# zarr-developers/zarr-python

Measured on AMD Instinct MI355X. Metric: decoded GiB/s (device-resident), sharded 256^3 f32 64^3 chunks, 1/2/4/8 GPU, higher is better.
Workload: dtype u8

## Files before the change

include/zarrhip.h:

```cpp
#ifndef ZARRHIP_H
#define ZARRHIP_H

#include <stdint.h>

#ifdef __cplusplus
extern "C" {
#endif

#define ZHIP_ABI_VERSION 1
#define ZHIP_MAX_DIMS 8

#define ZHIP_OK 0
#define ZHIP_E_INVALID -1
#define ZHIP_E_HIP -2
#define ZHIP_E_UNSUPPORTED -3
#define ZHIP_E_IO -4
#define ZHIP_E_BOUNDS -5

#define ZHIP_ST_OK 0u
#define ZHIP_ST_MISSING 1u
#define ZHIP_ST_CRC_MISMATCH 2u
#define ZHIP_ST_INDEX_OOB 3u
#define ZHIP_ST_LENGTH_MISMATCH 4u

// ... 377 lines not shown
typedef struct zhip_value_op {
    uint32_t encode;
    uint32_t array_dt;
    uint32_t stored_dt;
    uint32_t stages;
    uint64_t offset, scale;
    uint32_t rounding;
    uint32_t out_of_range;
    uint32_t n_map;
    uint32_t fill_nan;
    uint64_t map_key[ZHIP_VALUE_MAX_MAP];
    uint64_t map_val[ZHIP_VALUE_MAX_MAP];
    uint64_t fill;
} zhip_value_op;

#define ZHIP_VI_MISSING 1u
#define ZHIP_VI_STATUS 2u

typedef struct zhip_value_dim {
    int64_t sa, sb;
    uint32_t count;
    uint32_t _pad;
    zhip_fdiv div;
} zhip_value_dim;

typedef struct zhip_value_item {
    int64_t a_base, b_base;
    uint32_t ndim;
    uint32_t total;
    uint32_t flags;
    uint32_t status;
    zhip_value_dim dims[ZHIP_MAX_DIMS];
} zhip_value_item;

int zhip_value_map(const zhip_value_op *op, const zhip_value_item *d_items, uint32_t n_items,
                   const uint32_t *d_tile_prefix, uint32_t n_tiles, const zhip_status *d_status,
                   const void *a, uint64_t a_size, void *b, uint64_t b_size, uint32_t *d_err,
                   uint32_t *d_nonempty, void *stream);
int zhip_emulate_value_map(const zhip_value_op *op, const zhip_value_item *items, uint32_t n_items,
                           const uint32_t *tile_prefix, uint32_t n_tiles, const zhip_status *status,
                           uint32_t n_status, const void *a, uint64_t a_size, void *b, uint64_t b_size,
                           uint32_t *err, uint32_t *nonempty);

int zhip_emulate_fill_eq(uint32_t itemsize, uint32_t lflags, const void *fill, const void *items,
                         uint64_t n_items, uint8_t *eq, uint32_t *fill_nan);

uint32_t zhip_crc32c_host(const void *data, uint64_t nbytes);

int zhip_selftest(void);
uint32_t zhip_emulate_chunk_crc(const zhip_plan *plan, const uint8_t *data);
uint32_t zhip_emulate_chunk_crc_pair(const zhip_plan *plan, const uint8_t *data);
uint32_t zhip_emulate_chunk_crc_il(const zhip_plan *plan, const uint8_t *data);
uint32_t zhip_emulate_chunk_crc_xw(const zhip_plan *plan, const uint8_t *data);
uint64_t zhip_plan_table_image(const zhip_plan *plan, int which, uint32_t *out, uint64_t cap);
uint32_t zhip_plan_table_offsets(const zhip_plan *plan, uint64_t *out, uint32_t cap);
uint32_t zhip_fdiv_eval(uint32_t n, uint32_t d);

#ifdef __cplusplus
}
#endif

#endif
```

zarr-python_amd/csrc/capi.cpp:

```cpp
#include <hip/hip_runtime.h>

#include <algorithm>
#include <climits>
#include <cstdio>
#include <cstdlib>
#include <cstring>
#include <new>
#include <string>
#include <vector>

#include "../../include/zarrhip.h"
#include "zhip_gf2.h"
#include "zhip_internal.h"
#include "zhip_axis.h"
#include "zhip_fill_eq.h"
#include "zhip_points.h"
#include "zhip_select.h"
#include "zhip_values.h"

using namespace zhip;

namespace {

thread_local std::string g_err;
// ... 1228 lines not shown
                acc = ap(0, acc ^ w[0]) ^ ap(1, w[1]) ^ ap(2, w[2]) ^ ap(3, w[3]);
            }
            unit ^= gf_mul(acc, h[T.kthread.off + t]);
        }
        V ^= gf_mul(unit, h[T.kunit.off + s]);
    }
    return ~(gf_mul(V, plan->c_inv) ^ plan->c3);
}

uint32_t zhip_emulate_chunk_crc_pair(const zhip_plan* plan, const uint8_t* data) {
    auto mulx = [](uint32_t b) { return (b >> 1) ^ (kPoly & (0u - (b & 1u))); };
    auto lanemul3 = [&](uint32_t a, uint32_t k) {
        uint32_t m3[8], m2[4];
        const uint32_t k1 = mulx(k), k2 = mulx(k1);
        for (uint32_t v = 0; v < 8; ++v) m3[v] = ((v & 4u) ? k : 0u) ^ ((v & 2u) ? k1 : 0u) ^ ((v & 1u) ? k2 : 0u);
        for (uint32_t v = 0; v < 4; ++v) m2[v] = ((v & 2u) ? k : 0u) ^ ((v & 1u) ? k1 : 0u);
        uint32_t p = m3[a & 7u];
        for (int j = 1; j < 10; ++j) p = mulx(mulx(mulx(p))) ^ m3[(a >> (3 * j)) & 7u];
        return mulx(mulx(p)) ^ m2[a >> 30];
    };
    const std::vector<uint32_t> h = build_row_tables(*plan);
    const TabSet& S = plan->tl.pair;
    return emulate_lanes(plan, data, &h[S.tab.off], &h[S.klane.off], S.klane.n, plan->kblocks,
                         [&](int64_t i, int64_t k) {
                             return (int64_t)plan->E - (i / kThreads + 1) * plan->seg + kWgStride * k + 16 * (i % kThreads);
                         },
                         lanemul3);
}

uint32_t zhip_emulate_chunk_crc_il(const zhip_plan* plan, const uint8_t* data) {
    if (!plan || !plan->il_S) return 0xFFFFFFFFu;
    const IlChoice c = il_choose(*plan, 0);
    const int64_t S = c.S, K = kDefaultBlocks;
    const int64_t lo_frame = (int64_t)plan->E - (int64_t)plan->nseg * K * kWgStride;
    const std::vector<uint32_t> h = build_row_tables(*plan);
    return emulate_lanes(plan, data, &h[c.set->tab.off], &h[c.set->klane.off], c.set->klane.n, (uint32_t)K,
                         [&](int64_t i, int64_t k) {
                             const int64_t r = i / kThreads, st0 = (r / S) * S * K + r % S;
                             return lo_frame + kWgStride * (st0 + S * k) + 16 * (i % kThreads);
                         },
                         [](uint32_t a, uint32_t k) { return gf_mul(a, k); });
}

uint32_t zhip_emulate_chunk_crc_xw(const zhip_plan* plan, const uint8_t* data) {
    if (!plan || !plan->xw_P) return 0xFFFFFFFFu;
    const int64_t lo_frame = (int64_t)plan->E - (int64_t)plan->nseg * kDefaultBlocks * kWgStride;
    const std::vector<uint32_t> h = build_row_tables(*plan);
    const TabSet& S = plan->tl.xw;
    return emulate_lanes(plan, data, &h[S.tab.off], &h[S.klane.off], S.klane.n, kDefaultBlocks,
                         [&](int64_t i, int64_t k) { return lo_frame + 8192 * (i / 64) + 1024 * k + 16 * (i % 64); },
                         [](uint32_t a, uint32_t k) { return gf_mul(a, k); });
}

int zhip_selftest(void) {
    const uint32_t* g_T = byte_tables().T;
    bool seen[256] = {false};
    for (int i = 0; i < 256; ++i) seen[g_T[i] >> 24] = true;
    for (int i = 0; i < 256; ++i)
        if (!seen[i]) return set_err(1, "T top-byte map is not a bijection");
    uint32_t v = 0x12345678u;
    for (int it = 0; it < 1000; ++it) {
        v = v * 1664525u + 1013904223u;
        const uint32_t a = (v >> 8) ^ g_T[v & 255u];
        if (a != gf_mul(v, xpow8(1))) return set_err(2, "A_1 != multiply by x^8");
        if (gf_mul(gf_mul(v, xpow8(777)), xpow8_inv(777)) != v) return set_err(3, "x^-8n inverse wrong");
    }
    if (crc_bytewise((const uint8_t*)"123456789", 9) != 0xE3069283u) return set_err(4, "check value");
    const uint32_t ds[] = {1, 2, 3, 5, 7, 10, 15, 60, 64, 100, 255, 256, 1000, 4096, 65537, 1000003u};
    for (uint32_t d : ds) {
        const zhip_fdiv f = make_fdiv(d);
        uint32_t x = 1;
        for (int it = 0; it < 20000; ++it) {
            x = x * 1103515245u + 12345u;
            const uint32_t n = (it < 1000) ? (uint32_t)it : (x & 0x7FFFFFFFu);
            if (fdiv_apply(n, f.m, f.s) != n / d) return set_err(5, "fdiv wrong");
        }
        const uint32_t nmax = 0x7FFFFFFFu;
        if (fdiv_apply(nmax, f.m, f.s) != nmax / d) return set_err(5, "fdiv wrong at 2^31-1");
    }
    const uint64_t sizes[] = {0, 1, 3, 4, 15, 16, 17, 100, 4095, 4096, 4097, 32768, 32769, 100000, 262148};
    std::vector<uint8_t> buf(262148);
    uint32_t r = 7;
    for (auto& b : buf) {
        r = r * 1664525u + 1013904223u;
        b = (uint8_t)(r >> 24);
    }
    for (uint64_t n : sizes) {
        zhip_layout L{};
        L.ndim = 1;
        L.itemsize = 1;
        L.shape[0] = (int32_t)n;
        L.nbytes = n;
        zhip_plan* p = nullptr;
        if (zhip_plan_create(&L, &p) != ZHIP_OK) return 6;
        const uint32_t got = zhip_emulate_chunk_crc(p, buf.data());
        const uint32_t got_pair = zhip_emulate_chunk_crc_pair(p, buf.data());
        zhip_plan_destroy(p);
        if (got != crc_bytewise(buf.data(), n)) return set_err(7, "emulated kernel CRC wrong at n=" + std::to_string(n));
        if (got_pair != crc_bytewise(buf.data(), n))
            return set_err(8, "emulated pair-kernel CRC wrong at n=" + std::to_string(n));
    }
    return 0;
}

}
```

zarr-python_amd/csrc/decode.hip:

```cpp
#include <hip/hip_runtime.h>

#include "../../include/zarrhip.h"
#include "zhip_gf2.h"
#include "zhip_internal.h"
#include "zhip_dispatch.h"
#include "zhip_device.h"
#include "zhip_decode_common.h"
#include "zhip_arrival.h"

namespace zhip {

#if ZHIP_TUNING
int g_tune_max_grid = 0;
#endif

template <bool CRC, bool WRITE, bool FAST, int ITEM, int SWAP, int K = 8>
__global__ __launch_bounds__(kThreads) void k_decode(const DecodeParams p) {
    __shared__ uint32_t s_tab[CRC ? 16 * 256 : 1];
    __shared__ uint32_t s_red[2][kThreads / 64];
    const int t = threadIdx.x;
    uint32_t kth = 0;
    const bool crc_on = CRC && !(p.tune & kTuneSkipCrc);
    if constexpr (CRC) {
        const uint4* g = reinterpret_cast<const uint4*>(p.horner);
// ... 546 lines not shown
        return select_il_kernel_arm(L.crc, L.item, L.swap, g_tune_arm);
    if (tune & kTuneCfLookup) return select_il_kernel_cf(L.crc, L.item, L.swap);
    if (tune & kTuneIlLean) return select_il_kernel_lean(L.crc, L.item, L.swap);
    if (tune & (kTuneIlRegMul | kTuneIlOcc6))
        return select_il_kernel_regmul(L.crc, L.item, L.swap, (tune & kTuneIlOcc6) != 0);
    if (tune & (kTuneNoTables | kTuneNoRunEnd | kTuneNoPub | kTuneStamp))
        return select_il_kernel_tuned(L.crc, L.item, L.swap);
#endif
    return select_il_kernel(L.crc, L.item, L.swap, L.p.aff_ok != 0);
}

static KernelFn pick_pair_kernel(const Launch& L, int nu) {
#if ZHIP_TUNING
    const uint32_t tune = L.tune;
    if (nu == 2 && !(tune & (kTuneTrailingCrc | kTuneSplitChain))) {
        KernelFn fn = (tune & kTuneSkipCrc) ? select_pair_kernel(L.crc, L.item, L.swap, kPairNoLookups)
                      : (tune & (kTunePrio | kTuneDeferB))
                          ? select_pair_kernel(L.crc, L.item, L.swap,
                                               (tune & kTunePrio) && (tune & kTuneDeferB) ? kPairPrioDeferB
                                               : (tune & kTunePrio) ? kPairPrio : kPairDeferB)
                          : nullptr;
        if (fn) return fn;
    }
#endif
    return select_pair_kernel(L.crc, L.item, L.swap, nu == 2 ? kPairTwo : kPairSingle);
}

static bool takes_lead4(const Launch& L) {
    return L.p.nseg == 1u && L.p.E <= 4u * kWgStride && g_tune_arm != kArmNoLead4;
}

static bool takes_lead(const Launch& L) { return !L.crc && L.p.n_idx; }

static bool takes_interleaved(const Launch& L) {
    const DecodeParams& p = L.p;
    return p.il_S != 0 && L.crc && !(L.tune & (kTuneNoIl | kTuneSkipCrc | kTuneSingle | kTuneDuo)) &&
           ((L.tune & kTuneIl) || p.il_S >= 8u);
}

static bool takes_ilh(const Launch& L, bool il) {
    const DecodeParams& p = L.p;
    return il && p.ilh_klane && p.n_units <= kIlwMaxUnits && L.lb_ok && p.nseg <= 32u &&
           (g_tune_arm == kArmProduction || g_tune_arm == kArmIlhProduction) && (L.tune & ~kTuneStamp) == 0;
}

static bool takes_ilw512(const Launch& L, bool il) {
    const DecodeParams& p = L.p;
    return il && p.ilw_nt == 512u && p.n_units <= kIlwMaxUnits &&
           (g_tune_arm == kArmProduction || g_tune_arm == kArmRowMap || g_tune_arm == kArmIlw512Small ||
            ((g_tune_arm == kArmSplitPub || g_tune_arm == kArmLookBack) && p.aff_ok)) &&
           (L.tune & ~kTuneStamp) == 0;
}

static int launch_row_units(const Launch& L) {
    const DecodeParams& p = L.p;
    const uint32_t tune = L.tune;
    const bool crc = L.crc;
    if (takes_lead4(L)) return launch_lead4(L);
    if (takes_lead(L)) return launch_lead(L);
    const bool il = takes_interleaved(L);
#if ZHIP_TUNING
    int rc;
    if (launch_row_arm(L, il, rc)) return rc;
#endif
    if (takes_ilh(L, il))
        return fire(select_ilh_kernel(L.item, L.swap, true, p.aff_ok != 0), "k_decode_ilh",
                    unit_grid(p, 2u * p.n_units), kThreads, p, L.stream);
    if (takes_ilw512(L, il)) {
        const IlwForm form = g_tune_arm == kArmSplitPub ? kIlw512Split
                             : (g_tune_arm == kArmLookBack && L.lb_ok && p.nseg <= 64u) ? kIlw512LookBack : kIlw512;
        return fire(select_ilw_kernel(L.item, L.swap, form, false, p.aff_ok != 0), "k_decode_ilw512",
                    unit_grid(p, p.n_units), 512, p, L.stream);
    }
    if (il) return fire(pick_il_kernel(L), "k_decode_il", unit_grid(p, p.n_units), kThreads, p, L.stream);
    const int nu = (tune & kTuneSingle) ? 1 : 2;
    KernelFn fn = pick_pair_kernel(L, nu);
    if (!fn) return ZHIP_E_UNSUPPORTED;
    if ((tune & kTuneDuo) || (p.nseg > 32 && !(tune & (kTuneSingle | kTuneSkipCrc))))
        return fire(select_duo_kernel(crc, L.item, L.swap), "k_decode_duo",
                    unit_grid(p, (uint32_t)(((uint64_t)p.n_units + 1u) / 2u)), 2 * kThreads, p, L.stream);
    const uint32_t grid = unit_grid(p, (uint32_t)(((uint64_t)p.n_units + nu - 1u) / nu));
    return fire(fn, "k_decode_pair", grid, kThreads, with_xcd_runs(L, grid, nu == 2), L.stream);
}

static int launch_persistent(const Launch& L, KernelFn fn, const char* name) {
    uint32_t grid = L.p.n_units;
    if (fn && grid) {
        const uint32_t resident = (uint32_t)resident_grid(fn, L.max_grid);
        if (grid > resident) grid = resident;
    }
    return fire(fn, name, grid, kThreads, L.p, L.stream);
}

static int launch_tile4(const Launch& L) {
    const DecodeParams& p = L.p;
    const bool f4 = ZHIP_TUNING && p.t4f_tab != nullptr && L.crc;
    const bool w4 = !f4 && p.t4w_tab != nullptr && L.crc;
    if (w4 && ((p.t2w_kq && g_tune_arm != kArmTileFour && g_tune_arm != kArmTile1w) ||
               (g_tune_arm == kArmTile1w && p.t1w_kq))) {
        const bool one = g_tune_arm == kArmTile1w;
        const Tile2wForm form = one ? kT2wOne : g_tune_arm == kArmSplitPub ? kT2wSplit
                                : (g_tune_arm == kArmTile2wByteTab && p.tbt_tab) ? kT2wByteTab : kT2wTwo;
        DecodeParams q = p;
        q.t4w_kq = one ? p.t1w_kq : p.t2w_kq;
        return fire(select_tile2w_kernel(L.item, L.swap, form),
                    one ? "k_decode_tile1w" : form == kT2wSplit ? "k_decode_tile2ws"
// ... 18 lines not shown
    const bool gw = p.t4w_tab != nullptr && L.crc;
    const bool defer = p.defer != 0 && g_tune_arm != kArmDeferred;
    TilegwForm form = (gw && p.t2w_kq && g_tune_arm != kArmTileFour && g_tune_arm != kArmDeferred &&
                       g_tune_arm != kArmTilegLanes) ? kTgwTwo : kTgwFour;
    const bool two = form == kTgwTwo;
#if ZHIP_TUNING
    if (gw && g_tune_arm == kArmTilegLanes && p.tglt_kq) form = kTgwLanes;
    if (two && g_tune_arm == kArmTilegPacked) form = kTgwPacked;
    if (two && g_tune_arm == kArmTilegLookBack && L.lb_ok && p.n_groups <= 128u) form = kTgwLookBack;
    if (two && g_tune_arm == kArmTilegByteTab && p.tbt_tab) form = kTgwByteTab;
#endif
    KernelFn fn = gw ? select_tilegw_kernel(L.item, L.swap, defer, form)
                     : select_tileg_kernel(L.crc, L.item, L.swap, defer);
    const uint64_t grid = (uint64_t)p.n_chunks * p.n_groups * (two ? 2u : 1u);
    if (grid >= (1ull << 31)) return ZHIP_E_UNSUPPORTED;
    DecodeParams q = p;
    if (two) q.t4w_kq = p.t2w_kq;
    if (form == kTgwLanes) q.t4w_kq = p.tglt_kq;
    return fire(fn, !gw ? "k_decode_tileg" : form == kTgwPacked ? "k_decode_tileg2wp"
                    : form == kTgwLookBack ? "k_decode_tileg2w_lb" : form == kTgwByteTab ? "k_decode_tileg2w_bt"
                    : two ? "k_decode_tileg2w" : form == kTgwLanes ? "k_decode_tileglt" : "k_decode_tilegw",
                (uint32_t)grid, kThreads, q, L.stream);
}

static Launch make_launch(const DecodeParams& p, hipStream_t stream, int max_grid) {
    const bool crc = (p.lflags & ZHIP_LF_CRC) != 0;
    const bool lb_ok = p.n_chunks < (uint32_t)(max_grid / 8);
    if (g_tune_max_grid > 0) max_grid = g_tune_max_grid;
    return {p, stream, max_grid, ZHIP_TUNING ? p.tune : 0u, lb_ok, crc, item_mode(p.lflags, (int)p.g.itemsize),
            p.g.itemsize};
}

static bool takes_row_units(const Launch& L) {
    const DecodeParams& p = L.p;
    const bool lead_launch = !L.crc && p.n_idx != 0;
    return p.rows && p.rowmap && p.seg == (uint32_t)kWgStride * kDefaultBlocks &&
           (!(L.tune & kTunePersist) || lead_launch);
}

static bool takes_plain_il(const Launch& L) {
    if (!takes_row_units(L) || takes_lead4(L) || takes_lead(L)) return false;
    const bool il = takes_interleaved(L);
    if (!il || takes_ilh(L, il) || takes_ilw512(L, il)) return false;
    return g_tune_arm == kArmProduction && L.tune == 0u;
}

uint64_t g_launch_count = 0;

int launch_decode_multi(const DecodeParams* ps, const int* max_grid, uint32_t n, hipStream_t stream, bool dry) {
    if (n < 2u || n > (uint32_t)ZHIP_MULTI_MAX) return ZHIP_E_UNSUPPORTED;
    MultiParams m{};
    MultiFn fn = nullptr;
    uint64_t total = 0;
    for (uint32_t i = 0; i < n; ++i) {
        const Launch L = make_launch(ps[i], stream, max_grid[i]);
        if (!takes_plain_il(L)) return ZHIP_E_UNSUPPORTED;
        MultiFn f = select_il_multi_kernel(L.crc, L.item, L.swap, ps[i].aff_ok != 0);
        if (!f || (i && f != fn)) return ZHIP_E_UNSUPPORTED;
        fn = f;
        const uint32_t grid = unit_grid(ps[i], ps[i].n_units);
        if (grid == 0) return ZHIP_E_UNSUPPORTED;
        m.q[i] = ps[i];
        m.g0[i] = (uint32_t)total;
        total += grid;
        if (total > 0x7FFFFFFFull) return ZHIP_E_UNSUPPORTED;
    }
    for (uint32_t i = n; i <= (uint32_t)ZHIP_MULTI_MAX; ++i) m.g0[i] = (uint32_t)total;
    m.n = n;
    if (dry) return ZHIP_OK;
    return fire(fn, "k_decode_il", (uint32_t)total, kThreads, m, stream);
}

int launch_decode(const DecodeParams& p, hipStream_t stream, int max_grid) {
    const Launch L = make_launch(p, stream, max_grid);
    const bool crc = L.crc;
    if (takes_row_units(L)) return launch_row_units(L);
    if (p.rows)
        return launch_persistent(L, select_rows_kernel(crc, L.item, L.swap, (int)(p.seg / kWgStride)), "k_decode_rows");
    if (p.tq >= 0 && p.tile4) return launch_tile4(L);
    if (p.tq >= 0 && p.tile2) return launch_tile_pairs(L);
    if (p.tq >= 0 && p.tileg) return launch_tile_groups(L);
    if (p.tq >= 0) return launch_persistent(L, select_tile_kernel(crc, L.item, L.swap), "k_decode_tile");
    return launch_persistent(L, select_decode_kernel(crc, (p.lflags & ZHIP_LF_NO_WRITE) == 0, p.fast != 0, L.item,
                                                     L.swap, (int)(p.seg / kWgStride)), "k_decode");
}

}

extern "C" const char* zhip_last_kernel(void) { return zhip::g_last_kernel; }
extern "C" uint32_t zhip_last_grid(void) { return zhip::g_last_grid; }
extern "C" uint64_t zhip_launch_count(void) { return zhip::g_launch_count; }
```

zarr-python_amd/csrc/decode_rows.hip:

```cpp
#include <hip/hip_runtime.h>

#include "../../include/zarrhip.h"
#include "zhip_gf2.h"
#include "zhip_internal.h"
#include "zhip_dispatch.h"
#include "zhip_device.h"
#include "zhip_decode_common.h"
#include "zhip_arrival.h"

namespace zhip {

namespace {

typedef unsigned int zhip_v4u_a1 __attribute__((ext_vector_type(4), aligned(1)));
typedef __attribute__((address_space(1))) const zhip_v4u_a1 zhip_gv4u_a1;

typedef __attribute__((address_space(1))) const uint32_t zhip_gu32_a1 __attribute__((aligned(1)));

__device__ __forceinline__ uint32_t load_u32_any(const uint8_t* a) {
    return *(zhip_gu32_a1*)(reinterpret_cast<uintptr_t>(a));
}

__device__ __forceinline__ uint4 load16_any(const uint8_t* a) {
    const zhip_v4u_a1 w = *(zhip_gv4u_a1*)(reinterpret_cast<uintptr_t>(a));
// ... 2081 lines not shown
        m[h] = load_uniform<zhip_rowblk>(p.rowmap + ((size_t)U.sel * p.nseg + sidx) * K + (st % (uint32_t)K));
    }
    uint32_t stored = 0;
    if (CRC && ok) stored = load_trailer_uniform(U.cp, p.g.nbytes);
    if constexpr (CRC) {
        uint4* stt = reinterpret_cast<uint4*>(s_tab);
        stt[t] = tv0;
        stt[t + kThreads] = tv1;
        stt[t + 2 * kThreads] = tv2;
        stt[t + 3 * kThreads] = tv3;
        stt[t + 4 * kThreads] = tv4;
        stt[t + 5 * kThreads] = tv5;
        lanemul3_init(s_mul, t, kl);
        __syncthreads();
    }
    if (has) {
        uint8_t* sink = reinterpret_cast<uint8_t*>(g_rows_sink);
        const bool writes = ok || U.mode == ZHIP_ST_MISSING;
        uint8_t* const obase = p.out + U.out_off;
        const uint4 f = make_uint4(p.fill[0], p.fill[1], p.fill[2], p.fill[3]);
        const uint32_t rmask = (1u << p.row_shift) - 1u;
        Acc4 acc = {0u, 0u, 0u, 0u};
#pragma unroll
        for (int k = 0; k < K; ++k) {
            const zhip_rowblk& mk = m[k >> 2];
            const uint32_t o = 1024u * (uint32_t)(k & 3) + 16u * l;
            const uint32_t lane_row = o >> p.row_shift;
            const bool wr = writes && lane_row - mk.lo < mk.hi - mk.lo;
            const int64_t lane_off = (int64_t)lane_row * p.r_oy + (int64_t)(o & rmask);
            store_nt16(wr ? obase + mk.rel + lane_off : sink, ok ? swap_block<ITEM, SWAP>(A[k]) : f);
            if (CRC && ok) crc_block4(s_tab, acc, A[k]);
        }
        if constexpr (CRC) {
            uint32_t v = ok ? lanemul3(s_mul, t, fold4(s_tab, acc)) : 0u;
            v = wave_xor(v);
            if (ok && !(p.tune & kTuneNoPub))
                publish_xw(p, c, r, __builtin_amdgcn_readfirstlane(v), __builtin_amdgcn_readfirstlane(stored), l);
        }
        if (r == 0) unit_status_pair(p, U, CRC, (int)l);
    }
    if constexpr (CRC)
        for (uint32_t j = g; j < p.n_idx; j += G) verify_index_pair(p, j, t, kix, s_tab, s_red, j == g, ipre);
}

#if ZHIP_TUNING
KernelFn select_xw_kernel(bool crc, int item, int swap) {
    if (!crc) return nullptr;
    return for_item(item, swap, [](auto t) -> KernelFn {
        return k_decode_xw<true, decltype(t)::item, decltype(t)::swap>;
    });
}
#endif

KernelFn select_duo_kernel(bool crc, int item, int swap) {
    return for_item(item, swap, [&](auto t) -> KernelFn {
        using T = decltype(t);
        return crc ? k_decode_duo<true, T::item, T::swap> : k_decode_duo<false, T::item, T::swap>;
    });
}

KernelFn select_rows_kernel(bool crc, int item, int swap, int k) {
#if ZHIP_TUNING
    if (k == 4) {
        return headline_item(crc, item, swap) ? k_decode_rows<true, 4, false, 4> : nullptr;
    }
#endif
    if (k != 8) return nullptr;
    return for_item(item, swap, [&](auto t) -> KernelFn {
        using T = decltype(t);
        return crc ? k_decode_rows<true, T::item, T::swap> : k_decode_rows<false, T::item, T::swap>;
    });
}

}
```

zarr-python_amd/csrc/zhip_internal.h:

```cpp
#pragma once
#include <hip/hip_runtime.h>
#include <stdint.h>

#include "../../include/zarrhip.h"
#include "zhip_plan_tables.h"

namespace zhip {

constexpr int kThreads = 256;
constexpr int kWgStride = kThreads * 16;
constexpr int kDefaultBlocks = 8;
constexpr uint32_t kPubLine = 32;

struct Geom {
    int32_t ndim, itemsize;
    int32_t shape[ZHIP_MAX_DIMS];
    int64_t ostride[ZHIP_MAX_DIMS];
    zhip_fdiv dshape[ZHIP_MAX_DIMS];
    uint32_t nbytes;
    uint32_t row_bytes;
    zhip_fdiv drow;
};

struct TileEnt {
    uint32_t tbase, _pad;
    int64_t orel;
};

struct GroupEnt {
    uint32_t tbase;
    uint16_t rows, cols;
    int64_t orel;
    uint32_t ku, _pad;
};

constexpr int kPairT1 = 0, kPairT2 = 2048, kPairT3 = 4096, kPairA4 = 5120;
constexpr int kPairTabWords = 6144;
constexpr int kByteTabWords = 2048;
extern const char* g_last_kernel;
extern uint32_t g_last_grid;
constexpr uint32_t kIlwMaxUnits = 512;
constexpr int kIlBasisWords = 64;

struct PairHot {
    uint32_t n_units, nseg, n_idx, xcd_run;
    zhip_fdiv d_nseg, d_xcd, d_per;
    uint32_t pred, pred_per, E, seg;
    uint32_t tune, pad;
    uint64_t pred_base, pred_outer, pred_inner;
    uint64_t src, pair_tab, kpair11, kthread11;
    uint32_t il_S, n_chunks;
    uint64_t il_tab, il_klane, il_kidx;
};

struct DecodeParams {
    PairHot h;
    const uint8_t* src;
    uint64_t src_size;
    uint8_t* out;
    const zhip_chunk* chunks;
    const zhip_sel* sels;
    zhip_status* status;
    uint32_t* ws;
    uint32_t* errflag;
    const uint32_t* horner;
    uint32_t hx[4];
    uint32_t kq[32];
    const uint32_t* kthread;
    const uint32_t* kunit;
    const uint32_t* kpair;
    const uint32_t* pair_tab;
    const uint32_t* kpair11;
    const uint32_t* kthread11;
    uint32_t n_chunks, nseg, n_units;
    uint32_t c_inv, c3;
    uint32_t lflags;
    Geom g;
    uint32_t seg;
    uint32_t E;
    uint32_t index_size, n_inner;
    uint32_t fill[4];
    uint32_t fast;
    uint32_t tune;
    int32_t tq;
    uint32_t t_per_chunk, n_qb, n_cb;
    uint32_t sstride[ZHIP_MAX_DIMS];
    zhip_fdiv d_qb, d_cb;
    uint32_t tile4;
    uint32_t tile2;
    const uint32_t* tz;
    const uint32_t* kq4;
    const struct TileEnt* tmap;
    const uint32_t* t4f_tab;
    const uint32_t* t4f_kq;
// ... 280 lines not shown
int launch_dv_check(const zhip_dv_ref* d_refs, uint32_t n_refs, hipStream_t stream);
int debug_stamps(uint64_t* host_out, uint32_t n_wg);

using KernelFn = void (*)(const DecodeParams);
using EncodeFn = void (*)(const EncodeParams);
using MultiFn = void (*)(const MultiParams);

enum PairForm {
    kPairSingle = 1,
    kPairTwo = 2,
    kPairNoLookups = 5,
    kPairPrio = 6,
    kPairDeferB = 7,
    kPairPrioDeferB = 8,
    kPairLead = 9,
    kPairLead4 = 10,
    kPairLead8 = 11,
};
enum IlwForm {
    kIlw512 = 512,
    kIlw1024 = 1024,
    kIlw512Half = 513,
    kIlw512Split = 515,
    kIlw512LookBack = 516,
};
enum Tile2wForm {
    kT2wOne = 1,
    kT2wTwo = 2,
    kT2wSplit = 3,
    kT2wByteTab = 4,
};
enum TilegwForm {
    kTgwTwo = 2,
    kTgwFour = 4,
    kTgwLanes = 5,
    kTgwPacked = 6,
    kTgwLookBack = 7,
    kTgwByteTab = 8,
};
enum EncTilegForm {
    kEtgTwo = 2,
    kEtgFour = 4,
    kEtgFourSpread = 6,
    kEtgTwoSpread = 7,
    kEtgLookBack = 8,
    kEtgA4 = 9,
};

KernelFn select_rows_kernel(bool crc, int item, int swap, int k);
KernelFn select_pair_kernel(bool crc, int item, int swap, PairForm form);
KernelFn select_duo_kernel(bool crc, int item, int swap);
KernelFn select_il_kernel(bool crc, int item, int swap, bool aff);
MultiFn select_il_multi_kernel(bool crc, int item, int swap, bool aff);
KernelFn select_ilw_kernel(int item, int swap, IlwForm form, bool lmr, bool aff);
KernelFn select_ilh_kernel(int item, int swap, bool lb, bool aff);
#if ZHIP_TUNING
KernelFn select_il_kernel_lean(bool crc, int item, int swap);
KernelFn select_il_kernel_tuned(bool crc, int item, int swap);
KernelFn select_il_kernel_arm(bool crc, int item, int swap, int arm);
KernelFn select_il_kernel_cf(bool crc, int item, int swap);
KernelFn select_il_kernel_regmul(bool crc, int item, int swap, bool occ6);
KernelFn select_xw_kernel(bool crc, int item, int swap);
KernelFn select_ilq_kernel(int item, int swap, int nq, bool glds);
KernelFn select_ilc_kernel(int item, int swap);
KernelFn select_ilp_kernel(int item, int swap);
#endif
#if ZHIP_TUNING
KernelFn select_tile4f_kernel(int item, int swap);
#endif
KernelFn select_tile4_kernel(bool crc, int item, int swap);
KernelFn select_tile4w_kernel(int item, int swap);
KernelFn select_tile2w_kernel(int item, int swap, Tile2wForm form);
KernelFn select_tilegw_kernel(int item, int swap, bool defer, TilegwForm form);
KernelFn select_tileg_kernel(bool crc, int item, int swap, bool defer);
EncodeFn select_encode_tile4_kernel(bool crc, int item, int swap, bool two);
EncodeFn select_encode_tile_kernel(bool crc, int item, int swap);
EncodeFn select_encode_tileg_kernel(bool crc, int item, int swap, EncTilegForm form);

}

struct zhip_plan {
    zhip_layout layout;
    uint32_t kblocks;
    uint32_t seg;
    uint32_t nseg;
    uint32_t E;
    uint64_t R;
    uint32_t c_inv, c3;
    uint32_t hx[4];
    uint32_t kq[32];
    zhip_fdiv dshape[ZHIP_MAX_DIMS];
    uint32_t row_bytes;
    zhip_fdiv drow;
    uint32_t fill[4];
    int device;
    int max_grid;
    uint32_t* d_tables;
    uint32_t* d_tile_tables;
    zhip::TableLayout tl;
    int32_t tq;
    uint32_t t_per_chunk, n_qb, n_cb;
    uint32_t sstride[ZHIP_MAX_DIMS];
    uint32_t t_c_inv;
    uint32_t tile4;
    uint64_t tile4_step;
    uint32_t tile4f;
// ... 13 lines not shown
```

zarr-python_amd/zarr_hip/_native.py:

```python

from __future__ import annotations

import ctypes
import os

import numpy as np

MAX_DIMS = 8

ST_OK = 0
ST_MISSING = 1
ST_CRC_MISMATCH = 2
ST_INDEX_OOB = 3
ST_LENGTH_MISMATCH = 4

LF_CRC = 1
LF_SWAP = 2
LF_SHARDED = 4
LF_INDEX_START = 8
LF_NO_WRITE = 16
LF_FLOAT = 32
LF_COMPLEX = 64

CF_MISSING = 1
# ... 244 lines not shown
                              ctypes.c_uint32, ctypes.c_void_p, ctypes.c_void_p, ctypes.c_void_p,
                              ctypes.c_void_p, ctypes.c_uint32, ctypes.c_void_p]
    L.zhip_encode.restype = ctypes.c_int
    L.zhip_encode_mapped.argtypes = L.zhip_encode.argtypes[:-1] + [ctypes.c_void_p, ctypes.c_void_p]
    L.zhip_encode_mapped.restype = ctypes.c_int
    L.zhip_shard_pack.argtypes = [ctypes.c_void_p, ctypes.c_void_p, ctypes.c_void_p, ctypes.c_uint32,
                                  ctypes.c_uint32, ctypes.c_uint32, ctypes.c_uint32, ctypes.c_uint32,
                                  ctypes.c_void_p, ctypes.c_void_p, ctypes.c_void_p, ctypes.c_void_p,
                                  ctypes.c_void_p]
    L.zhip_shard_pack.restype = ctypes.c_int
    L.zhip_set_tuning.argtypes = [ctypes.c_int, ctypes.c_int]
    L.zhip_set_tuning.restype = ctypes.c_int
    L.zhip_last_kernel.argtypes = []
    L.zhip_last_kernel.restype = ctypes.c_char_p
    L.zhip_last_grid.argtypes = []
    L.zhip_last_grid.restype = ctypes.c_uint32
    L.zhip_debug_stamps.argtypes = [ctypes.c_void_p, ctypes.c_uint32]
    L.zhip_debug_stamps.restype = ctypes.c_int
    L.zhip_selftest.restype = ctypes.c_int
    L.zhip_emulate_chunk_crc.argtypes = [ctypes.c_void_p, ctypes.c_void_p]
    L.zhip_emulate_chunk_crc.restype = ctypes.c_uint32
    L.zhip_stage_h2d.argtypes = [ctypes.c_void_p, ctypes.c_uint32, ctypes.c_void_p, ctypes.c_void_p,
                                 ctypes.c_uint64, ctypes.c_uint64, ctypes.c_uint32, ctypes.c_void_p]
    L.zhip_stage_h2d.restype = ctypes.c_int
    L.zhip_stage_begin.argtypes = list(L.zhip_stage_h2d.argtypes)
    L.zhip_stage_begin.restype = ctypes.c_void_p
    L.zhip_stage_end.argtypes = [ctypes.c_void_p, ctypes.c_void_p]
    L.zhip_stage_end.restype = ctypes.c_int
    L.zhip_host_pinned.argtypes = [ctypes.c_void_p]
    L.zhip_host_pinned.restype = ctypes.c_int
    L.zhip_wait_words.argtypes = [ctypes.c_void_p, ctypes.c_uint32, ctypes.c_void_p, ctypes.c_void_p]
    L.zhip_wait_words.restype = ctypes.c_int
    L.zhip_wait_ranges.argtypes = [ctypes.c_void_p, ctypes.c_void_p, ctypes.c_uint32, ctypes.c_void_p,
                                   ctypes.c_void_p]
    L.zhip_wait_ranges.restype = ctypes.c_int
    L.zhip_upload.argtypes = [ctypes.c_void_p, ctypes.c_void_p, ctypes.c_void_p, ctypes.c_uint32, ctypes.c_void_p,
                              ctypes.c_uint64, ctypes.c_void_p]
    L.zhip_upload.restype = ctypes.c_int
    L.zhip_dv_check.argtypes = [ctypes.c_void_p, ctypes.c_uint32, ctypes.c_void_p]
    L.zhip_dv_check.restype = ctypes.c_int
    vp, u32, u64 = ctypes.c_void_p, ctypes.c_uint32, ctypes.c_uint64
    L.zhip_plan_batch.argtypes = [vp, vp, u32, vp, vp, u64, vp, vp, u32, vp, vp, vp, vp, vp, vp]
    L.zhip_plan_batch.restype = ctypes.c_int
    L.zhip_crc32c_host.argtypes = [ctypes.c_void_p, ctypes.c_uint64]
    L.zhip_crc32c_host.restype = ctypes.c_uint32
    L.zhip_host_copy.argtypes = [ctypes.c_void_p, ctypes.c_void_p, ctypes.c_uint64, ctypes.c_uint32]
    L.zhip_host_copy.restype = ctypes.c_int
    L.zhip_emulate_chunk_crc_pair.argtypes = [ctypes.c_void_p, ctypes.c_void_p]
    L.zhip_emulate_chunk_crc_pair.restype = ctypes.c_uint32
    L.zhip_emulate_chunk_crc_il.argtypes = [ctypes.c_void_p, ctypes.c_void_p]
    L.zhip_emulate_chunk_crc_il.restype = ctypes.c_uint32
    L.zhip_emulate_chunk_crc_xw.argtypes = [ctypes.c_void_p, ctypes.c_void_p]
    L.zhip_emulate_chunk_crc_xw.restype = ctypes.c_uint32
    L.zhip_plan_table_image.argtypes = [ctypes.c_void_p, ctypes.c_int, ctypes.c_void_p, ctypes.c_uint64]
    L.zhip_plan_table_image.restype = ctypes.c_uint64
    L.zhip_plan_table_offsets.argtypes = [ctypes.c_void_p, ctypes.c_void_p, ctypes.c_uint32]
    L.zhip_plan_table_offsets.restype = ctypes.c_uint32
    L.zhip_fdiv_eval.argtypes = [ctypes.c_uint32, ctypes.c_uint32]
    L.zhip_fdiv_eval.restype = ctypes.c_uint32
    L.zhip_tuning_build.restype = ctypes.c_int
    L.zhip_select_copy.argtypes = [vp, u32, vp, vp, u32, vp, u64, vp, u64, u32, vp]
    L.zhip_select_copy.restype = ctypes.c_int
    L.zhip_emulate_select_copy.argtypes = [vp, u32, vp, u64, vp, u32, vp, u64, vp, u64, u32]
    L.zhip_emulate_select_copy.restype = ctypes.c_int
    L.zhip_value_map.argtypes = [vp, vp, u32, vp, u32, vp, vp, u64, vp, u64, vp, vp, vp]
    L.zhip_value_map.restype = ctypes.c_int
    L.zhip_emulate_value_map.argtypes = [vp, vp, u32, vp, u32, vp, u32, vp, u64, vp, u64, vp, vp]
    L.zhip_emulate_value_map.restype = ctypes.c_int
    L.zhip_points_count.argtypes = [vp, vp, u64, vp, vp, vp]
    L.zhip_points_count.restype = ctypes.c_int
    L.zhip_points_fill.argtypes = [vp, vp, u64, vp, vp, vp, vp]
    L.zhip_points_fill.restype = ctypes.c_int
    L.zhip_emulate_points.argtypes = [vp, vp, u64, vp, vp, vp, vp, vp]
    L.zhip_emulate_points.restype = ctypes.c_int
    L.zhip_axis_last.argtypes = [vp, vp, u64, vp, vp]
    L.zhip_axis_last.restype = ctypes.c_int
    L.zhip_axis_count.argtypes = [vp, vp, u64, vp, vp, vp, vp, vp, vp]
    L.zhip_axis_count.restype = ctypes.c_int
    L.zhip_axis_fill.argtypes = [vp, vp, u64, vp, vp, vp, vp, u64, vp]
    L.zhip_axis_fill.restype = ctypes.c_int
    L.zhip_emulate_axis.argtypes = [vp, vp, u64, ctypes.c_int, vp, vp, vp, vp, vp, vp, vp, vp, u64]
    L.zhip_emulate_axis.restype = ctypes.c_int
    L.zhip_emulate_fill_eq.argtypes = [u32, u32, vp, vp, u64, vp, vp]
    L.zhip_emulate_fill_eq.restype = ctypes.c_int
    if L.zhip_abi_version() != 1:
        raise NativeError("libzarrhip ABI version mismatch")
    if L.zhip_tuning_build() and not _override_allowed():
        raise NativeError(f"{LIB_PATH} is the tuning build (measurement arms compiled in): it loads only with "
                          f"{OVERRIDE_OPT_IN}=1")
    _lib = L
    return L


def tuning_build() -> bool:
    return bool(lib().zhip_tuning_build())


def check(rc: int, what: str) -> None:
    if rc != 0:
        msg = lib().zhip_last_error().decode(errors="replace")
        raise NativeError(f"{what} failed ({rc}): {msg}")


def fdiv(d: int) -> tuple[int, int]:
    d = max(int(d), 1)
    l = (d - 1).bit_length()
    s = 31 + l
    m = ((1 << s) + d - 1) // d
    return m, s


class Plan:

    def __init__(self, layout: Layout, upload: bool = True):
        self.layout = layout
        h = ctypes.c_void_p()
        check(lib().zhip_plan_create(ctypes.byref(layout), ctypes.byref(h)), "zhip_plan_create")
        self._h = h
        upc = ctypes.c_uint32()
        wsw = ctypes.c_uint32()
        check(lib().zhip_plan_info(h, ctypes.byref(upc), ctypes.byref(wsw)), "zhip_plan_info")
        self.units_per_chunk = upc.value
        self.workspace_words = wsw.value
        if upload:
            check(lib().zhip_plan_upload(h), "zhip_plan_upload")

    @property
    def handle(self):
        return self._h

    @property
    def kernel_flags(self) -> int:
        f = ctypes.c_uint32()
        check(lib().zhip_plan_kernel_flags(self._h, ctypes.byref(f)), "zhip_plan_kernel_flags")
        return f.value

    def emulate_chunk_crc(self, data: bytes, pair: bool = False) -> int:
        buf = ctypes.create_string_buffer(bytes(data) + b"\0" * 16)
        fn = lib().zhip_emulate_chunk_crc_il if pair == "il" else lib().zhip_emulate_chunk_crc_xw if pair == "xw" else \
            lib().zhip_emulate_chunk_crc_pair if pair else lib().zhip_emulate_chunk_crc
        return int(fn(self._h, buf))

    def table_image(self, which: int) -> np.ndarray:
        n = int(lib().zhip_plan_table_image(self._h, which, None, 0))
        out = np.zeros(n, np.uint32)
        assert int(lib().zhip_plan_table_image(self._h, which, out.ctypes.data, n)) == n
        return out

    def table_regions(self) -> tuple[list[int], list[int]]:
        n = int(lib().zhip_plan_table_offsets(self._h, None, 0))
        out = np.zeros(2 * n, np.uint64)
        assert int(lib().zhip_plan_table_offsets(self._h, out.ctypes.data, 2 * n)) == n
        return [int(v) for v in out[:n]], [int(v) for v in out[n:]]

    def __del__(self):
        h = getattr(self, "_h", None)
        if h and _lib is not None:
            _lib.zhip_plan_destroy(h)
            self._h = None
```

Before: 2687.

## Add full-row interleaved multi-GPU decode kernel covering four spans per block

Adds a new decode kernel in which each workgroup processes four consecutive 8 KiB spans of a row for four chunks, one chunk per wave. It uses a combined lane multiplier taken from the last span, so it publishes one CRC partial per four spans. The multi-launch path selects it when every shard has many units, a span count divisible by four, and a chunk count divisible by four. The aim is to cut per-block overhead (table loads, index resolution, publishes) and the total block count, at the cost of higher register pressure and fewer, larger blocks. A host emulator for the new CRC lane composition is added for testing.

```diff
diff --git a/include/zarrhip.h b/include/zarrhip.h
--- a/include/zarrhip.h
+++ b/include/zarrhip.h
@@ -453,6 +453,7 @@
 uint32_t zhip_emulate_chunk_crc_pair(const zhip_plan *plan, const uint8_t *data);
 uint32_t zhip_emulate_chunk_crc_il(const zhip_plan *plan, const uint8_t *data);
 uint32_t zhip_emulate_chunk_crc_xw(const zhip_plan *plan, const uint8_t *data);
+uint32_t zhip_emulate_chunk_crc_ilx(const zhip_plan *plan, const uint8_t *data, uint32_t P);
 uint64_t zhip_plan_table_image(const zhip_plan *plan, int which, uint32_t *out, uint64_t cap);
 uint32_t zhip_plan_table_offsets(const zhip_plan *plan, uint64_t *out, uint32_t cap);
 uint32_t zhip_fdiv_eval(uint32_t n, uint32_t d);
diff --git a/zarr-python_amd/csrc/capi.cpp b/zarr-python_amd/csrc/capi.cpp
--- a/zarr-python_amd/csrc/capi.cpp
+++ b/zarr-python_amd/csrc/capi.cpp
@@ -1304,6 +1304,19 @@
                          [](uint32_t a, uint32_t k) { return gf_mul(a, k); });
 }
 
+uint32_t zhip_emulate_chunk_crc_ilx(const zhip_plan* plan, const uint8_t* data, uint32_t P) {
+    if (!plan || !plan->xw_P || P == 0 || plan->xw_P % P) return 0xFFFFFFFFu;
+    const int64_t lo_frame = (int64_t)plan->E - (int64_t)plan->nseg * kDefaultBlocks * kWgStride;
+    const std::vector<uint32_t> h = build_row_tables(*plan);
+    const TabSet& S = plan->tl.xw;
+    const uint64_t n_lanes = (uint64_t)(plan->xw_P / P) * 64;
+    std::vector<uint32_t> kl(n_lanes);
+    for (uint64_t i = 0; i < n_lanes; ++i) kl[i] = h[S.klane.off + ((i / 64) * P + (P - 1)) * 64 + i % 64];
+    return emulate_lanes(plan, data, &h[S.tab.off], kl.data(), n_lanes, kDefaultBlocks * P,
+                         [&](int64_t i, int64_t k) { return lo_frame + 8192 * (i / 64) * (int64_t)P + 1024 * k + 16 * (i % 64); },
+                         [](uint32_t a, uint32_t k) { return gf_mul(a, k); });
+}
+
 int zhip_selftest(void) {
     const uint32_t* g_T = byte_tables().T;
     bool seen[256] = {false};
diff --git a/zarr-python_amd/csrc/decode.hip b/zarr-python_amd/csrc/decode.hip
--- a/zarr-python_amd/csrc/decode.hip
+++ b/zarr-python_amd/csrc/decode.hip
@@ -622,6 +622,17 @@
            (L.tune & ~kTuneStamp) == 0;
 }
 
+static bool takes_fullrow(const Launch& L, bool il) {
+    const DecodeParams& p = L.p;
+    return il && L.crc && p.xw != 0 && p.xw % kIlxSpans == 0u && p.xw / kIlxSpans <= 32u &&
+           p.n_units > kIlwMaxUnits && p.n_chunks % 4u == 0u && g_tune_arm == kArmProduction && L.tune == 0u;
+}
+
+static uint64_t fullrow_grid(const DecodeParams& p) {
+    const uint64_t g = (uint64_t)(p.n_chunks / 4u) * (p.xw / kIlxSpans);
+    return g > p.n_idx ? g : p.n_idx;
+}
+
 static int launch_row_units(const Launch& L) {
     const DecodeParams& p = L.p;
     const uint32_t tune = L.tune;
@@ -746,13 +757,19 @@
     MultiParams m{};
     MultiFn fn = nullptr;
     uint64_t total = 0;
+    bool fr = true;
     for (uint32_t i = 0; i < n; ++i) {
         const Launch L = make_launch(ps[i], stream, max_grid[i]);
         if (!takes_plain_il(L)) return ZHIP_E_UNSUPPORTED;
-        MultiFn f = select_il_multi_kernel(L.crc, L.item, L.swap, ps[i].aff_ok != 0);
+        fr = fr && takes_fullrow(L, true);
+    }
+    for (uint32_t i = 0; i < n; ++i) {
+        const Launch L = make_launch(ps[i], stream, max_grid[i]);
+        MultiFn f = fr ? select_ilx_multi_kernel(L.crc, L.item, L.swap, ps[i].aff_ok != 0)
+                       : select_il_multi_kernel(L.crc, L.item, L.swap, ps[i].aff_ok != 0);
         if (!f || (i && f != fn)) return ZHIP_E_UNSUPPORTED;
         fn = f;
-        const uint32_t grid = unit_grid(ps[i], ps[i].n_units);
+        const uint32_t grid = fr ? (uint32_t)fullrow_grid(ps[i]) : unit_grid(ps[i], ps[i].n_units);
         if (grid == 0) return ZHIP_E_UNSUPPORTED;
         m.q[i] = ps[i];
         m.g0[i] = (uint32_t)total;
diff --git a/zarr-python_amd/csrc/decode_rows.hip b/zarr-python_amd/csrc/decode_rows.hip
--- a/zarr-python_amd/csrc/decode_rows.hip
+++ b/zarr-python_amd/csrc/decode_rows.hip
@@ -2157,6 +2157,157 @@
 }
 #endif
 
+template <bool CRC, int ITEM, int SWAP, bool AFF>
+__device__ __forceinline__ void ilx_body(const DecodeParams& p, const uint32_t g, const uint32_t G) {
+    constexpr int K = kDefaultBlocks, NP = (int)kIlxSpans;
+    if constexpr (AFF) __builtin_amdgcn_s_setprio(3);
+    __shared__ uint32_t s_tab[CRC ? kPairTabWords : 1];
+    __shared__ uint32_t s_mul[CRC ? 12 * kThreads : 1];
+    __shared__ uint32_t s_red[kThreads / 64];
+    const int t = threadIdx.x;
+    const uint32_t l = (uint32_t)t & 63u;
+    const uint32_t wv = __builtin_amdgcn_readfirstlane((uint32_t)t >> 6);
+    const uint32_t wpc = p.xw / (uint32_t)NP;
+    const uint32_t quad = g / wpc, r = g - quad * wpc;
+    if (quad * 4u >= p.n_chunks && g >= p.n_idx) return;
+    const uint32_t c = quad * 4u + wv;
+    const bool has = c < p.n_chunks;
+    const uint32_t expected = p.g.nbytes + (CRC ? 4u : 0u);
+    const uint8_t* zero = reinterpret_cast<const uint8_t*>(g_rows_zero);
+    uint4 tv0, tv1, tv2, tv3, tv4, tv5;
+    uint32_t kl = 0, kix = 0;
+    if constexpr (CRC) {
+        const uint4* gt = reinterpret_cast<const uint4*>(p.xw_tab);
+        tv0 = gt[t];
+        tv1 = gt[t + kThreads];
+        tv2 = gt[t + 2 * kThreads];
+        tv3 = gt[t + 3 * kThreads];
+        tv4 = gt[t + 4 * kThreads];
+        tv5 = gt[t + 5 * kThreads];
+        kl = load_u32_any(reinterpret_cast<const uint8_t*>(p.xw_klane + ((size_t)r * NP + (NP - 1)) * 64u + l));
+        kix = load_u32_any(reinterpret_cast<const uint8_t*>(p.xw_kidx + t));
+    }
+    Unit U;
+    if (has) U = resolve_unit(p, c * p.nseg, expected);
+    else {
+        U.c = 0;
+        U.sidx = 0;
+        U.mode = ZHIP_ST_MISSING;
+        U.cp = zero;
+        U.seg_lo = 0;
+        U.sel = 0;
+        U.out_off = 0;
+    }
+    const bool ok = has && U.mode == ZHIP_ST_OK;
+    const int32_t lo_frame = (int32_t)p.E - (int32_t)(p.nseg * p.seg);
+    const int32_t span0 = lo_frame + 8192 * (int32_t)(r * (uint32_t)NP);
+    uint4 ipre = make_uint4(0, 0, 0, 0);
+    if constexpr (CRC) ipre = index_prefetch(p, g, g < p.n_idx, t, zero);
+    uint4 A[K];
+#pragma unroll
+    for (int k = 0; k < K; ++k) {
+        const int32_t base = span0 + 1024 * k;
+        A[k] = load_stream16_any(ok && base >= 0 ? U.cp + base + 16 * l : zero);
+    }
+    if constexpr (AFF) __builtin_amdgcn_s_setprio(0);
+    zhip_rowblk m[2 * NP];
+    if (AFF && (!has || sel_whole(p, U.sel))) {
+#pragma unroll
+        for (int h = 0; h < 2 * NP; ++h) m[h] = aff_rowblk(p, 2u * (uint32_t)NP * r + (uint32_t)h);
+    } else {
+#pragma unroll
+        for (int h = 0; h < 2 * NP; ++h) {
+            const uint32_t st = 2u * (uint32_t)NP * r + (uint32_t)h;
+            const uint32_t sidx = p.nseg - 1u - st / (uint32_t)K;
+            m[h] = load_uniform<zhip_rowblk>(p.rowmap + ((size_t)U.sel * p.nseg + sidx) * K + (st % (uint32_t)K));
+        }
+    }
+    uint32_t stored = 0;
+    if (CRC && ok) stored = load_trailer_uniform(U.cp, p.g.nbytes);
+    if constexpr (CRC) {
+        uint4* stt = reinterpret_cast<uint4*>(s_tab);
+        stt[t] = tv0;
+        stt[t + kThreads] = tv1;
+        stt[t + 2 * kThreads] = tv2;
+        stt[t + 3 * kThreads] = tv3;
+        stt[t + 4 * kThreads] = tv4;
+        stt[t + 5 * kThreads] = tv5;
+        lanemul3_init(s_mul, t, kl);
+        __syncthreads();
+    }
+    if (has) {
+        uint8_t* sink = reinterpret_cast<uint8_t*>(g_rows_sink);
+        const bool writes = ok || U.mode == ZHIP_ST_MISSING;
+        uint8_t* const obase = p.out + U.out_off;
+        const uint4 f = make_uint4(p.fill[0], p.fill[1], p.fill[2], p.fill[3]);
+        const uint32_t rmask = (1u << p.row_shift) - 1u;
+        Acc4 acc = {0u, 0u, 0u, 0u};
+#pragma unroll
+        for (int pp = 0; pp < NP; ++pp) {
+            if (pp != 0) {
+#pragma unroll
+                for (int k = 0; k < K; ++k) {
+                    const int32_t base = span0 + 8192 * pp + 1024 * k;
+                    A[k] = load_stream16_any(ok && base >= 0 ? U.cp + base + 16 * l : zero);
+                }
+            }
+#pragma unroll
+            for (int k = 0; k < K; ++k) {
+                const zhip_rowblk& mk = m[2 * pp + (k >> 2)];
+                const uint32_t o = 1024u * (uint32_t)(k & 3) + 16u * l;
+                const uint32_t lane_row = o >> p.row_shift;
+                const bool wr = writes && lane_row - mk.lo < mk.hi - mk.lo;
+                const int64_t lane_off = (int64_t)lane_row * p.r_oy + (int64_t)(o & rmask);
+                store_nt16(wr ? obase + mk.rel + lane_off : sink, ok ? swap_block<ITEM, SWAP>(A[k]) : f);
+                if (CRC && ok) crc_block4(s_tab, acc, A[k]);
+            }
+        }
+        if constexpr (CRC) {
+            uint32_t v = ok ? lanemul3(s_mul, t, fold4(s_tab, acc)) : 0u;
+            v = wave_xor(v);
+            if (ok)
+                publish_il(p, c, r, wpc, __builtin_amdgcn_readfirstlane(v), __builtin_amdgcn_readfirstlane(stored),
+                           (int)l, kPubLine / 2u);
+        }
+        if (r == 0) unit_status_pair(p, U, CRC, (int)l);
+    }
+    if constexpr (CRC)
+        for (uint32_t j = g; j < p.n_idx; j += G) verify_index_pair(p, j, t, kix, s_tab, s_red, j == g, ipre);
+}
+
+template <bool CRC, int ITEM, int SWAP, bool AFF>
+__global__ __launch_bounds__(kThreads) __attribute__((amdgpu_waves_per_eu(4, 4)))
+void k_decode_ilx(const DecodeParams p) {
+    ilx_body<CRC, ITEM, SWAP, AFF>(p, blockIdx.x, gridDim.x);
+}
+
+template <bool CRC, int ITEM, int SWAP, bool AFF>
+__global__ __launch_bounds__(kThreads) __attribute__((amdgpu_waves_per_eu(4, 4)))
+void k_decode_ilx_multi(const MultiParams m) {
+    const uint32_t b = blockIdx.x;
+    uint32_t i = 0;
+#pragma unroll
+    for (uint32_t k = 1; k < ZHIP_MULTI_MAX; ++k) i += (k < m.n && b >= m.g0[k]) ? 1u : 0u;
+    ilx_body<CRC, ITEM, SWAP, AFF>(m.q[i], b - m.g0[i], m.g0[i + 1] - m.g0[i]);
+}
+
+KernelFn select_ilx_kernel(bool crc, int item, int swap, bool aff) {
+    if (!crc) return nullptr;
+    return for_item(item, swap, [&](auto t) -> KernelFn {
+        using T = decltype(t);
+        return aff ? k_decode_ilx<true, T::item, T::swap, true> : k_decode_ilx<true, T::item, T::swap, false>;
+    });
+}
+
+MultiFn select_ilx_multi_kernel(bool crc, int item, int swap, bool aff) {
+    if (!crc) return nullptr;
+    return for_item(item, swap, [&](auto t) -> MultiFn {
+        using T = decltype(t);
+        return aff ? k_decode_ilx_multi<true, T::item, T::swap, true>
+                   : k_decode_ilx_multi<true, T::item, T::swap, false>;
+    });
+}
+
 KernelFn select_duo_kernel(bool crc, int item, int swap) {
     return for_item(item, swap, [&](auto t) -> KernelFn {
         using T = decltype(t);
diff --git a/zarr-python_amd/csrc/zhip_internal.h b/zarr-python_amd/csrc/zhip_internal.h
--- a/zarr-python_amd/csrc/zhip_internal.h
+++ b/zarr-python_amd/csrc/zhip_internal.h
@@ -40,6 +40,7 @@
 extern const char* g_last_kernel;
 extern uint32_t g_last_grid;
 constexpr uint32_t kIlwMaxUnits = 512;
+constexpr uint32_t kIlxSpans = 4;
 constexpr int kIlBasisWords = 64;
 
 struct PairHot {
@@ -426,6 +427,8 @@
 KernelFn select_duo_kernel(bool crc, int item, int swap);
 KernelFn select_il_kernel(bool crc, int item, int swap, bool aff);
 MultiFn select_il_multi_kernel(bool crc, int item, int swap, bool aff);
+KernelFn select_ilx_kernel(bool crc, int item, int swap, bool aff);
+MultiFn select_ilx_multi_kernel(bool crc, int item, int swap, bool aff);
 KernelFn select_ilw_kernel(int item, int swap, IlwForm form, bool lmr, bool aff);
 KernelFn select_ilh_kernel(int item, int swap, bool lb, bool aff);
 #if ZHIP_TUNING
diff --git a/zarr-python_amd/zarr_hip/_native.py b/zarr-python_amd/zarr_hip/_native.py
--- a/zarr-python_amd/zarr_hip/_native.py
+++ b/zarr-python_amd/zarr_hip/_native.py
@@ -320,6 +320,8 @@
     L.zhip_emulate_chunk_crc_il.restype = ctypes.c_uint32
     L.zhip_emulate_chunk_crc_xw.argtypes = [ctypes.c_void_p, ctypes.c_void_p]
     L.zhip_emulate_chunk_crc_xw.restype = ctypes.c_uint32
+    L.zhip_emulate_chunk_crc_ilx.argtypes = [ctypes.c_void_p, ctypes.c_void_p, ctypes.c_uint32]
+    L.zhip_emulate_chunk_crc_ilx.restype = ctypes.c_uint32
     L.zhip_plan_table_image.argtypes = [ctypes.c_void_p, ctypes.c_int, ctypes.c_void_p, ctypes.c_uint64]
     L.zhip_plan_table_image.restype = ctypes.c_uint64
     L.zhip_plan_table_offsets.argtypes = [ctypes.c_void_p, ctypes.c_void_p, ctypes.c_uint32]
@@ -409,6 +411,10 @@
             lib().zhip_emulate_chunk_crc_pair if pair else lib().zhip_emulate_chunk_crc
         return int(fn(self._h, buf))
 
+    def emulate_chunk_crc_fullrow(self, data: bytes, spans: int) -> int:
+        buf = ctypes.create_string_buffer(bytes(data) + b"\0" * 16)
+        return int(lib().zhip_emulate_chunk_crc_ilx(self._h, buf, spans))
+
     def table_image(self, which: int) -> np.ndarray:
         n = int(lib().zhip_plan_table_image(self._h, which, None, 0))
         out = np.zeros(n, np.uint32)
```

Result: faster. 2765 (median of 6 runs) (+2.9%).
